# shichaoy/cube_slam

Hardware: AMD Instinct MI355X
Metric: frames/sec front-end (ORB extract + LSD+LBD lines + cuboid: Canny+DT+sweep+score+select) @640x480 (higher is better)
Workload: dtype f64

## Files before the change

### cube_slam_amd/csrc/cuboid.hip

```cpp
#include "common.h"

#include <algorithm>
#include <array>
#include <climits>
#include <cmath>
#include <vector>

namespace {

constexpr int ROLL_CAP = 8;
constexpr int RP_CAP = ROLL_CAP * ROLL_CAP;
constexpr int SWEEP_HB = 1024;
constexpr int NMS_TW = 64, NMS_TH = 16;
constexpr int DT_INIT = INT_MAX >> 2;
constexpr int DT_HV = 62587;
constexpr int DT_DIAG = 89738;
constexpr size_t DT_SERIAL_ROW_BYTES = 2 * 4 * sizeof(int);
constexpr double PI = 3.14159265358979323846;
constexpr int SC_LDS_BYTES = 160 * 1024;
constexpr int SC_LUT_N = 1024;
constexpr int SC_CTRL_BYTES = 64;
constexpr int SC_MAP_OFF = SC_CTRL_BYTES + 2048;
constexpr int SC_MAP_ENTRIES = (SC_LDS_BYTES - SC_MAP_OFF) / 2;
constexpr float SC_ESC_D = 244.0f;
// ... 824 lines not shown
}

__device__ __forceinline__ void hyp_decode(const Unit &U, int h, int &q, int &ti) {
    const unsigned p = (unsigned)h >> 1;
    q = U.tops_magic ? (int)__umulhi(p, U.tops_magic) : (int)(p / (unsigned)U.n_tops);
    ti = (int)p - q * U.n_tops;
}

__device__ __forceinline__ V2 hit_vertical(V2 ps, V2 pe, double bx, double by0, double by1) {
    const double dx = pe.x - ps.x, dy = pe.y - ps.y;
    const double lambd = (bx - ps.x) / dx;
    const double ty = ps.y + lambd * dy;
    const bool hit = lambd >= 0 && by0 <= ty && ty <= by1;
    return V2{hit ? bx : -1.0, hit ? ty : -1.0};
}
__device__ __forceinline__ V2 hit_horizontal(V2 ps, V2 pe, double by, double bx0, double bx1) {
    const double dx = pe.x - ps.x, dy = pe.y - ps.y;
    const double lambd = (by - ps.y) / dy;
    const double tx = ps.x + lambd * dx;
    const bool hit = lambd >= 0 && bx0 <= tx && tx <= bx1;
    return V2{hit ? tx : -1.0, hit ? by : -1.0};
}

template <bool TESTS, bool N78>
__device__ __forceinline__ int corners_build(const Unit &U, const double *vp, int top_x, int cfg, V2 (&c)[8], bool live = true) {
    auto short_edge = [](V2 a, V2 b) { const double dx = a.x - b.x, dy = a.y - b.y; return dx * dx + dy * dy < __longlong_as_double(0x4078ffffffffffffll); };
    const V2 vp_1{vp[0], vp[1]}, vp_2{vp[2], vp[3]}, vp_3{vp[4], vp[5]};
    const double left = U.left, right = U.right, top = U.top, down = U.down_y_expan;
    const V2 c1{(double)top_x, top};
    const V2 c2r = hit_vertical(vp_1, c1, right, top, down), c2l = hit_vertical(vp_1, c1, left, top, down);
    const int pos = c2r.x != -1 ? 1 : (c2l.x != -1 ? 2 : 0);
    const V2 c2 = pos == 1 ? c2r : c2l;
    bool alive = live && pos > 0;
    if (TESTS) { alive = alive && !short_edge(c1, c2); if (!__any(alive)) return 0; }
    const bool k1 = cfg == 1;
    const V2 S = k1 ? c1 : c2, other = k1 ? c2 : c1;
    const V2 X = hit_vertical(vp_2, S, pos == 1 ? left : right, top, down);
    if (TESTS) { alive = alive && X.y != -1 && !short_edge(S, X); if (!__any(alive)) return 0; }
    const V2 Y = k1 ? line_intersect_inf(vp_2, other, vp_1, X) : line_intersect_inf(vp_1, X, vp_2, other);
    if (TESTS) {
        alive = alive && inside_box(Y, left, k1 ? top : (double)U.roi_y, right, k1 ? down : (double)U.roi_b) && !short_edge(Y, X) && !short_edge(Y, other);
        if (!__any(alive)) return 0;
    }
    const V2 c3 = k1 ? Y : X, c4 = k1 ? X : Y;
    const double el = U.roi_x, et = U.roi_y, er = U.roi_r, eb = U.roi_b;
    const V2 c5 = hit_horizontal(vp_3, c3, down, left, right);
    if (TESTS) { alive = alive && c5.y != -1 && !short_edge(c3, c5); if (!__any(alive)) return 0; }
    const V2 c6 = line_intersect_inf(vp_2, c5, vp_3, c2);
    if (TESTS) { alive = alive && inside_box(c6, el, et, er, eb) && !short_edge(c6, c2) && !short_edge(c6, c5); if (!__any(alive)) return 0; }
    c[0] = c1; c[1] = c2; c[2] = c3; c[3] = c4; c[4] = c5; c[5] = c6;
    if (TESTS || N78) {
        const V2 c7 = line_intersect_inf(vp_1, c6, vp_3, c1);
        if (TESTS) { alive = alive && inside_box(c7, el, et, er, eb) && !short_edge(c7, c1) && !short_edge(c7, c6); if (!__any(alive)) return 0; }
        const V2 c8 = line_intersect_inf(vp_1, c5, vp_2, c7);
        if (TESTS) alive = alive && inside_box(c8, el, et, er, eb) && !short_edge(c8, c4) && !short_edge(c8, c5) && !short_edge(c8, c7);
        c[6] = c7; c[7] = c8;
    } else { c[6] = V2{0, 0}; c[7] = V2{0, 0}; }
    return alive ? pos : 0;
}

__global__ void __launch_bounds__(256) cuboid_sweep_filter(const Unit *units, const int *wg_unit, const FrameDyn *fd, Opts o,
                                                           const VPEntry *vpt, uint8_t *flag, int *vcount, int *vlist) {
    __shared__ int s_list[2][SWEEP_HB / 2];
    __shared__ int s_wc[2][SWEEP_HB / 64];
    __shared__ int s_base[2];
    const int u = __builtin_amdgcn_readfirstlane(wg_unit[blockIdx.x]);
    const Unit &U = units[u];
// ... 314 lines not shown
        k = s_misc[1];
    }
    return prefix;
}
template <class P, class F> __device__ int block_ordered_visit(int n, P pred, F cb, int *s_wave ) {
    const int lane = threadIdx.x & 63, wave = threadIdx.x >> 6, nw = blockDim.x >> 6;
    int running = 0;
    for (int base = 0; base < n; base += blockDim.x) {
        int i = base + threadIdx.x;
        bool p = i < n && pred(i);
        unsigned long long m = __ballot(p);
        if (lane == 0) s_wave[wave] = __popcll(m);
        __syncthreads();
        int off = running, tot = 0;
        for (int w2 = 0; w2 < nw; w2++) { int c = s_wave[w2]; if (w2 < wave) off += c; tot += c; }
        if (p) cb(i, off + __popcll(m & ((1ull << lane) - 1)));
        running += tot;
        __syncthreads();
    }
    return running;
}

struct Conv3D { double pos[3], scale[3]; };
__device__ inline void plane_hit(const double *T, const double *invK, const double *pl, double px, double py, double *o3) {
    double ray[3];
    for (int i = 0; i < 3; i++) {
        double s = invK[i * 3] * px;
        s = s + invK[i * 3 + 1] * py;
        s = s + invK[i * 3 + 2] * 1.0;
        ray[i] = s;
    }
    double den = pl[0] * ray[0];
    den = den + pl[1] * ray[1];
    den = den + pl[2] * ray[2];
    double frac = -pl[3] / den;
    double s4[4] = {frac * ray[0], frac * ray[1], frac * ray[2], 1.0};
    double w[4];
    for (int i = 0; i < 4; i++) {
        double a = T[i * 4] * s4[0];
        a = a + T[i * 4 + 1] * s4[1];
        a = a + T[i * 4 + 2] * s4[2];
        a = a + T[i * 4 + 3] * s4[3];
        w[i] = a;
    }
    o3[0] = w[0] / w[3]; o3[1] = w[1] / w[3]; o3[2] = w[2] / w[3];
}
__device__ inline void corners_to_3d(const double *cx, const double *cy, const CamRP &C, const double *invK, Conv3D &o) {
    double g[4][3];
    for (int i = 0; i < 4; i++) plane_hit(C.T, invK, C.gps, cx[4 + i], cy[4 + i], g[i]);
    auto nrm = [](const double *a, const double *b) {
        double dx = a[0] - b[0], dy = a[1] - b[1], dz = a[2] - b[2];
        return sqrt(dx * dx + dy * dy + dz * dz);
    };
    double length_half = nrm(g[0], g[3]) / 2;
    double width_half = nrm(g[0], g[1]) / 2;
    double d[3] = {g[0][0] - g[1][0], g[0][1] - g[1][1], g[0][2] - g[1][2]};
    double nw[3] = {d[1] * 1.0 - d[2] * 0.0, d[2] * 0.0 - d[0] * 1.0, d[0] * 0.0 - d[1] * 0.0};
    double nn = sqrt(nw[0] * nw[0] + nw[1] * nw[1] + nw[2] * nw[2]);
    nw[0] /= nn; nw[1] /= nn; nw[2] /= nn;
    double dist = -((nw[0] * g[0][0] + nw[1] * g[0][1]) + nw[2] * g[0][2]);
    double pw[4] = {nw[0], nw[1], nw[2], dist};
    if (dist < 0) for (int i = 0; i < 4; i++) pw[i] = -pw[i];
    double ps[4];
    for (int i = 0; i < 4; i++) {
        double s = C.T[0 * 4 + i] * pw[0];
        s = s + C.T[1 * 4 + i] * pw[1];
        s = s + C.T[2 * 4 + i] * pw[2];
        s = s + C.T[3 * 4 + i] * pw[3];
        ps[i] = s;
    }
    double top[3];
    plane_hit(C.T, invK, ps, cx[1], cy[1], top);
    double height_half = top[2] / 2;
    o.pos[0] = (((g[0][0] + g[1][0]) + g[2][0]) + g[3][0]) / 4.0;
    o.pos[1] = (((g[0][1] + g[1][1]) + g[2][1]) + g[3][1]) / 4.0;
    o.pos[2] = height_half;
    o.scale[0] = length_half; o.scale[1] = width_half; o.scale[2] = height_half;
}

#ifndef SELECT_WAVES
#define SELECT_WAVES 3
#endif
__global__ void __launch_bounds__(256) __attribute__((amdgpu_waves_per_eu(SELECT_WAVES, SELECT_WAVES))) cuboid_select(const Unit *units, UnitDyn *ud, const int *box_first_unit, const FrameDyn *fd,
                                                     const FrameInfo *fi, const CamRP *cam, const double *yaw, Calib cal, Opts o,
                                                     uint8_t *flag, const double *derr, const double *aerr, const VPEntry *vpt,
                                                     double *score, double *nscore, unsigned long long *ckey_d, unsigned long long *ckey_a,
                                                     int *cidx, cs_cuboid *out, int *counts, int *carry_rp) {
    __shared__ int hist[256];
    __shared__ int s_last;
    __shared__ int s_misc[8];
    __shared__ int s_wave[8];
    __shared__ double s_red[4][4];
    __shared__ double s_best[4];
    __shared__ int s_bi[4][2];
    __shared__ int s_branch[4];
    const int box = blockIdx.x, tid = threadIdx.x, lane = tid & 63, wave = tid >> 6;
    const int u0 = box_first_unit[box];
    const int n_hs = units[u0].n_hs;
    const FrameDyn &D = fd[units[u0].frame];
    const FrameInfo &FI = fi[units[u0].frame];
    const int n_rp = D.n_roll * D.n_pitch;
    const double weight_vp_angle = 0.8, weight_skew_error = 1.5;
    int n_cand_total = 0;

    for (int hs = 0; hs < n_hs; hs++) {
        const int u = u0 + hs;
        const Unit &U = units[u];
        const int n_hyp = n_rp * D.n_yaw * U.n_tops * 2;
        uint8_t *fl = flag + U.hyp_off;
        const double *de = derr + U.hyp_off, *ae = aerr + U.hyp_off;
        unsigned long long *ckd = ckey_d + U.hyp_off, *cka = ckey_a + U.hyp_off;
        int *ch = cidx + U.hyp_off;
        const int n = block_ordered_visit(n_hyp, [&](int i) { return fl[i] != 0; },
                                          [&](int i, int r) { ckd[r] = dkey(de[i]); cka[r] = dkey(ae[i]); ch[r] = i; }, s_wave);
        __syncthreads();
        KeyCache kd, ka;
#pragma unroll
        for (int k = 0; k < SEL_R; k++) { int e = tid + 256 * k; kd.v[k] = e < n ? ckd[e] : 0; ka.v[k] = e < n ? cka[e] : 0; }
        int branch_b = 0, n_kept = 0;
        if (tid == 0) s_last = n - 1;
        if (n > 4) {
            int breaking_num = (int)round(float(n) / 3.0 * 2.0);
            int k = breaking_num - 1;
            unsigned long long vd = block_select_kth(kd, ckd, n, k - 1, hist, s_misc);
            unsigned long long va = block_select_kth(ka, cka, n, k - 1, hist, s_misc);
            unsigned long long va1 = block_select_kth(ka, cka, n, k, hist, s_misc);
            __syncthreads();
            if (tid == 0) { s_misc[2] = 0; s_misc[3] = 0; s_misc[4] = INT_MAX; }
            __syncthreads();
            {
                int nl = 0, ne = 0;
                for_keys(kd, ckd, n, [&](unsigned long long key, int) { nl += key < vd; ne += key == vd; });
                for (int off = 32; off > 0; off >>= 1) { nl += __shfl_xor(nl, off); ne += __shfl_xor(ne, off); }
                if (lane == 0) { atomicAdd(&s_misc[2], nl); atomicAdd(&s_misc[3], ne); }
            }
            __syncthreads();
            const int need_eq = k - s_misc[2];
            if (need_eq < s_misc[3] && tid == 0) {
                int seen = 0;
                for (int e = 0; e < n; e++) if (ckd[e] == vd && ++seen == need_eq) { s_misc[4] = e; break; }
            }
            __syncthreads();
            const int e_star = s_misc[4];
            const bool use_angle = va1 > va;
            if (!use_angle) branch_b = 1;
#pragma unroll
            for (int kk = 0; kk < SEL_R; kk++) {
                int e = tid + 256 * kk;
                if (e < n) {
                    bool ok = kd.v[kk] < vd || (kd.v[kk] == vd && e <= e_star);
                    if (use_angle) ok = ok && ka.v[kk] <= va;
                    if (ok) fl[ch[e]] |= 4;
                }
            }
            for (int e = tid + 256 * SEL_R; e < n; e += 256) {
                bool ok = ckd[e] < vd || (ckd[e] == vd && e <= e_star);
                if (use_angle) ok = ok && cka[e] <= va;
                if (ok) fl[ch[e]] |= 4;
            }
            if (hs == n_hs - 1 && carry_rp) {
                __syncthreads();
                if (tid == 0) s_last = -1;
                __syncthreads();
                int mine = -1;
                for (int e = tid; e < n; e += 256) {
                    const bool kept = (ckd[e] < vd || (ckd[e] == vd && e <= e_star)) && (!use_angle || cka[e] <= va);
                    if (kept && (use_angle || ckd[e] == vd)) mine = e;
                }
                if (mine >= 0) atomicMax(&s_last, mine);
                __syncthreads();
            }
        } else {
            for (int e = tid; e < n; e += 256) fl[ch[e]] |= 4;
        }
        __syncthreads();
        if (hs == n_hs - 1 && carry_rp) {
            __syncthreads();
            if (tid == 0) {
                int rp = n_rp - 1;
                if (n > 0 && s_last >= 0) { int q, ti; hyp_decode(U, ch[s_last], q, ti); rp = q / D.n_yaw; }
                carry_rp[box] = rp;
            }
        }
        double mn_d = 1e6, mx_d = -1, mn_a = 1e6, mx_a = -1;
        int cntk = 0;
        for (int e = tid; e < n; e += 256) {
            const int i = ch[e];
            if (fl[i] & 4) {
                double td = de[i], ta = ae[i];
                mn_d = fmin(mn_d, td); mx_d = fmax(mx_d, td); mn_a = fmin(mn_a, ta); mx_a = fmax(mx_a, ta);
                cntk++;
            }
        }
        for (int off = 32; off > 0; off >>= 1) {
            mn_d = fmin(mn_d, __shfl_xor(mn_d, off)); mx_d = fmax(mx_d, __shfl_xor(mx_d, off));
            mn_a = fmin(mn_a, __shfl_xor(mn_a, off)); mx_a = fmax(mx_a, __shfl_xor(mx_a, off));
            cntk += __shfl_xor(cntk, off);
        }
        if (lane == 0) { s_red[wave][0] = mn_d; s_red[wave][1] = mx_d; s_red[wave][2] = mn_a; s_red[wave][3] = mx_a; s_wave[wave] = cntk; }
        __syncthreads();
        mn_d = fmin(fmin(s_red[0][0], s_red[1][0]), fmin(s_red[2][0], s_red[3][0]));
        mx_d = fmax(fmax(s_red[0][1], s_red[1][1]), fmax(s_red[2][1], s_red[3][1]));
        mn_a = fmin(fmin(s_red[0][2], s_red[1][2]), fmin(s_red[2][2], s_red[3][2]));
        mx_a = fmax(fmax(s_red[0][3], s_red[1][3]), fmax(s_red[2][3], s_red[3][3]));
        n_kept = s_wave[0] + s_wave[1] + s_wave[2] + s_wave[3];
        __syncthreads();
        int ncand = 0;
        for (int e = tid; e < n; e += 256) {
            const int i = ch[e];
            if (!(fl[i] & 4)) continue;
            double dk = de[i], ak = ae[i], comb;
            if (n_kept > 1) {
                comb = (dk - mn_d) / (mx_d - mn_d);
                if ((mx_a - mn_a) > 0) ak = (ak - mn_a) / (mx_a - mn_a);
                comb = (comb + weight_vp_angle * ak) / (1 + weight_vp_angle);
            } else
                comb = (dk + weight_vp_angle * ak) / (1 + weight_vp_angle);
            long g = U.hyp_off + i;
            int q, ti;
            hyp_decode(U, i, q, ti);
            int rp = q / D.n_yaw;
            double cx[8], cy[8];
            {
                V2 c[8];
                corners_build<false, true>(U, vpt[(long)U.vp_off + q].vp, U.top_start + ti * U.top_step, (i & 1) + 1, c);
                for (int k = 0; k < 8; k++) { cx[k] = c[k].x; cy[k] = c[k].y; }
            }
            Conv3D c3;
            corners_to_3d(cx, cy, cam[(long)U.frame * RP_CAP + rp], cal.invK, c3);
            if (c3.scale[0] < 0 || c3.scale[1] < 0 || c3.scale[2] < 0) continue;
            double mxs = c3.scale[0] < c3.scale[1] ? c3.scale[1] : c3.scale[0];
            double mns = c3.scale[1] < c3.scale[0] ? c3.scale[1] : c3.scale[0];
            double skew_ratio = mxs / mns;
            double dsk = skew_ratio - o.nominal_skew_ratio;
            double skew_error = weight_skew_error * ((dsk < 0.0) ? 0.0 : dsk);
            if (skew_ratio > o.max_cut_skew) skew_error = 100;
            nscore[g] = comb;
            score[g] = comb + weight_skew_error * skew_error;
            fl[i] |= 8;
            ncand++;
        }
        for (int off = 32; off > 0; off >>= 1) ncand += __shfl_xor(ncand, off);
        if (lane == 0) s_wave[wave] = ncand;
        __syncthreads();
        n_cand_total += s_wave[0] + s_wave[1] + s_wave[2] + s_wave[3];
        if (tid == 0) { ud[u].n_valid = n; ud[u].n_kept = n_kept; ud[u].branch_b = branch_b; s_branch[hs] = branch_b; }
        __syncthreads();
    }

    const int kout = n_cand_total < o.max_cuboid_num ? n_cand_total : o.max_cuboid_num;
    for (int pick = 0; pick < kout; pick++) {
        double bs = 0, bd = 0; int bhs = -1, bi = -1;
        for (int hs = 0; hs < n_hs; hs++) {
            const Unit &U = units[u0 + hs];
            const int n_hyp = n_rp * D.n_yaw * U.n_tops * 2;
            const uint8_t *fl = flag + U.hyp_off;
            const int bb = s_branch[hs];
            for (int i = tid; i < n_hyp; i += 256) {
                if (!(fl[i] & 8)) continue;
                double s = score[U.hyp_off + i], dd = bb ? derr[U.hyp_off + i] : 0.0;
                bool better = bi < 0 || s < bs || (s == bs && (hs < bhs || (hs == bhs && (dd < bd || (dd == bd && i < bi)))));
                if (better) { bs = s; bd = dd; bhs = hs; bi = i; }
            }
        }
        for (int off = 32; off > 0; off >>= 1) {
            double s2 = __shfl_xor(bs, off), d2 = __shfl_xor(bd, off);
            int hs2 = __shfl_xor(bhs, off), i2 = __shfl_xor(bi, off);
            bool better = i2 >= 0 && (bi < 0 || s2 < bs || (s2 == bs && (hs2 < bhs || (hs2 == bhs && (d2 < bd || (d2 == bd && i2 < bi))))));
            if (better) { bs = s2; bd = d2; bhs = hs2; bi = i2; }
        }
        if (lane == 0) { s_best[wave] = bs; s_red[wave][0] = bd; s_bi[wave][0] = bhs; s_bi[wave][1] = bi; }
        __syncthreads();
        if (tid == 0) {
            for (int w2 = 1; w2 < 4; w2++) {
                double s2 = s_best[w2], d2 = s_red[w2][0];
                int hs2 = s_bi[w2][0], i2 = s_bi[w2][1];
                bool better = i2 >= 0 && (bi < 0 || s2 < bs || (s2 == bs && (hs2 < bhs || (hs2 == bhs && (d2 < bd || (d2 == bd && i2 < bi))))));
                if (better) { bs = s2; bd = d2; bhs = hs2; bi = i2; }
            }
            const Unit &U = units[u0 + bhs];
            long g = U.hyp_off + bi;
            flag[g] &= ~8;
            int cfg = (bi & 1) + 1, q, ti;
            hyp_decode(U, bi, q, ti);
            int yi = q % D.n_yaw, rp = q / D.n_yaw;
            const CamRP &C = cam[(long)U.frame * RP_CAP + rp];
            double cx[8], cy[8];
            {
                V2 c[8];
                corners_build<false, true>(U, vpt[(long)U.vp_off + q].vp, U.top_start + ti * U.top_step, cfg, c);
                for (int k = 0; k < 8; k++) { cx[k] = c[k].x; cy[k] = c[k].y; }
            }
            Conv3D c3;
            corners_to_3d(cx, cy, C, cal.invK, c3);
            cs_cuboid &O = out[(long)box * o.max_cuboid_num + pick];
            for (int k = 0; k < 3; k++) { O.pos[k] = c3.pos[k]; O.scale[k] = c3.scale[k]; }
            O.rotY = yaw[(long)U.frame * o.yaw_cap + yi];
            int vp1 = flag[g] & 3;
            O.box_config_type[0] = cfg; O.box_config_type[1] = vp1;
            const int map1[8] = {6, 5, 8, 7, 2, 3, 4, 1}, map2[8] = {5, 6, 7, 8, 3, 2, 1, 4};
            for (int k = 0; k < 8; k++) {
                int src = (vp1 == 1 ? map1[k] : map2[k]) - 1;
// ... 17 lines not shown
                    for (int i = 0; i < 3; i++) {
                        double s = rs[i][0] * body[0][k];
                        s = s + rs[i][1] * body[1][k];
                        s = s + rs[i][2] * body[2][k];
                        s = s + O.pos[i] * 1.0;
                        wv[i] = s;
                    }
                    wv[3] = ((0.0 * body[0][k] + 0.0 * body[1][k]) + 0.0 * body[2][k]) + 1.0;
                    for (int i = 0; i < 3; i++) O.box_corners_3d_world[i * 8 + k] = wv[i] / wv[3];
                }
            }
            O.rect_detect_2d[0] = U.left; O.rect_detect_2d[1] = U.top; O.rect_detect_2d[2] = U.width_raw; O.rect_detect_2d[3] = U.height_raw;
            O.edge_distance_error = derr[g]; O.edge_angle_error = aerr[g];
            O.normalized_error = nscore[g];
            double mxs = c3.scale[0] < c3.scale[1] ? c3.scale[1] : c3.scale[0];
            double mns = c3.scale[1] < c3.scale[0] ? c3.scale[1] : c3.scale[0];
            O.skew_ratio = mxs / mns;
            O.down_expand_height = U.down_expand;
            if (o.sample_rp) { O.camera_roll_delta = C.roll - FI.euler[0]; O.camera_pitch_delta = C.pitch - FI.euler[1]; }
            else { O.camera_roll_delta = 0; O.camera_pitch_delta = 0; }
        }
        __syncthreads();
    }
    if (tid == 0) counts[box] = kout;
}

__global__ void cuboid_bgr2gray(const uint8_t *bgr, int stride, int w, int h, uint8_t *gray) {
    int x = blockIdx.x * blockDim.x + threadIdx.x, y = blockIdx.y;
    if (x >= w) return;
    const uint8_t *p = bgr + (long)y * stride + 3 * x;
    gray[(long)y * w + x] = (uint8_t)((p[0] * 1868 + p[1] * 9617 + p[2] * 4899 + 8192) >> 14);
}

static void host_euler_from_T(const double *T, double *euler) {
    double m[3][3];
    for (int i = 0; i < 3; i++) for (int j = 0; j < 3; j++) m[i][j] = T[i * 4 + j];
    double qw, qx, qy, qz, q[3];
    double t = m[0][0] + m[1][1] + m[2][2];
    if (t > 0) {
        t = std::sqrt(t + 1.0);
        qw = 0.5 * t; t = 0.5 / t;
        qx = (m[2][1] - m[1][2]) * t; qy = (m[0][2] - m[2][0]) * t; qz = (m[1][0] - m[0][1]) * t;
    } else {
        int i = 0;
        if (m[1][1] > m[0][0]) i = 1;
        if (m[2][2] > m[i][i]) i = 2;
        int j = (i + 1) % 3, k = (j + 1) % 3;
// ... 140 lines not shown
    cs_pinned<uint8_t> stage[2]; hipEvent_t stage_ev[2] = {nullptr, nullptr}; int stage_k = 0;
    hipEvent_t ev_fork = nullptr, ev_join = nullptr;
    int score_G = 256;
    int score_T = 512;
    bool score_T_forced = false;
    bool want_carry = false;
    uint8_t *d_gray = nullptr;
    FrameInfo *d_fi = nullptr; FrameDyn *d_fd = nullptr; CamRP *d_cam = nullptr;
    double *d_yaw = nullptr;
    int *d_status = nullptr, *d_cursor = nullptr;
    uint8_t *d_emap = nullptr, *d_flag = nullptr;
    float *d_dist = nullptr;
    int *d_lab = nullptr;
    int *d_dttmp = nullptr; long *d_dttmp_off = nullptr;
    int *d_wgmap = nullptr;
    int *d_order = nullptr;
    int *d_uflag = nullptr;
    double *d_lines_in = nullptr, *d_lines_al = nullptr, *d_mlines = nullptr, *d_mangle = nullptr, *d_mmid = nullptr;
    Unit *d_units = nullptr; UnitDyn *d_ud = nullptr; int *d_box_first = nullptr, *d_counts = nullptr, *d_carry = nullptr;
    VPEntry *d_vp = nullptr;
    int *d_vcount = nullptr, *d_vlist = nullptr;
    double *d_derr = nullptr, *d_aerr = nullptr, *d_score = nullptr, *d_nscore = nullptr;
    unsigned long long *d_ckd = nullptr, *d_cka = nullptr; int *d_cidx = nullptr;
    cs_cuboid *d_out = nullptr;
    cs_cuboid_batch() { cap.fill(-1); }
};
static void plan_commit(cs_cuboid_batch *b, Plan &P) { static_cast<Plan &>(*b) = std::move(P); }

struct BatchArray { void **slot; int cls; size_t elem, mul, add; };
template <class T> static BatchArray array_of(T *&p, int cls, size_t mul = 1, size_t add = 0) { return {reinterpret_cast<void **>(&p), cls, sizeof(T), mul, add}; }
constexpr size_t N_BATCH_ARRAYS = 29;
static std::array<BatchArray, N_BATCH_ARRAYS> batch_arrays(cs_cuboid_batch *b) {
    return {{array_of(b->d_emap, K_PIX, 1, 256),
             array_of(b->d_dist, K_PIX),
             array_of(b->d_flag, K_HYP), array_of(b->d_vlist, K_HYP), array_of(b->d_derr, K_HYP), array_of(b->d_aerr, K_HYP), array_of(b->d_score, K_HYP), array_of(b->d_nscore, K_HYP),
             array_of(b->d_ckd, K_HYP), array_of(b->d_cka, K_HYP), array_of(b->d_cidx, K_HYP),
             array_of(b->d_vp, K_VP),
             array_of(b->d_units, K_UNITS), array_of(b->d_ud, K_UNITS), array_of(b->d_order, K_UNITS), array_of(b->d_uflag, K_UNITS), array_of(b->d_vcount, K_UNITS, 2),
             array_of(b->d_dttmp_off, K_UNITS, 1, 1),
             array_of(b->d_box_first, K_BOXES), array_of(b->d_counts, K_BOXES), array_of(b->d_carry, K_BOXES), array_of(b->d_out, K_BOXES, (size_t)b->o.max_cuboid_num),
             array_of(b->d_lines_in, K_LINES_IN, 4), array_of(b->d_lines_al, K_LINES_IN, 4),
             array_of(b->d_mlines, K_LINE_ROWS, 4), array_of(b->d_mangle, K_LINE_ROWS), array_of(b->d_mmid, K_LINE_ROWS, 2),
             array_of(b->d_wgmap, K_WGMAP),
             array_of(b->d_dttmp, K_DTTMP)}};
}
static int batch_reserve(cs_ctx *ctx, cs_cuboid_batch *b, const Needs &need, bool exact) {
    Needs cap = b->cap;
    for (int c = 0; c < K_N; c++)
        if (need[c] > cap[c]) cap[c] = exact ? need[c] : need[c] + need[c] / 4 + (c == K_LINES_IN || c == K_LINE_ROWS ? 64 : 0);
    if (cap == b->cap) return CS_OK;
    const auto arrays = batch_arrays(b);
    cs_owner fresh;
    std::array<uint8_t *, N_BATCH_ARRAYS> blk{};
    for (size_t i = 0; i < arrays.size(); i++) {
        const BatchArray &A = arrays[i];
        if (cap[A.cls] == b->cap[A.cls]) continue;
        const int r = fresh.alloc(ctx, &blk[i], std::max<size_t>(1, (size_t)cap[A.cls] * A.mul + A.add) * A.elem);
        if (r != CS_OK) { fresh.free_all(ctx); return r; }
    }
    bool replaces = false;
    for (size_t i = 0; i < arrays.size(); i++) replaces |= blk[i] && *arrays[i].slot;
    const hipError_t e = replaces ? ctx->drain() : hipSuccess;
// ... 213 lines not shown
    if (fork) { CS_HIP(ctx, hipEventRecord(b->ev_join, side)); branch.joined = b->ev_join; }
    CS_HIP(ctx, hipMemsetAsync(b->d_emap, 0, (size_t)b->pix_total, ctx->stream));
    CS_LAUNCH(ctx, "cuboid_canny_nms", cuboid_canny_nms, dim3(b->n_nms), dim3(256), 0, b->d_units, b->d_wgmap, b->d_gray, b->W, b->H, b->d_emap,
              b->d_lab, b->o.canny_low, b->o.canny_high);
    CS_LAUNCH(ctx, "cuboid_canny_cc_local", cuboid_canny_cc_local, dim3(b->n_cc), dim3(256), 0, b->d_units, b->d_wgmap + b->n_nms, b->d_emap, b->d_lab);
    if (b->max_cc_blocks > 1)
        CS_LAUNCH(ctx, "cuboid_canny_cc_border", cuboid_canny_cc_border, dim3(U, 4), dim3(256), 0, b->d_units, b->d_emap, b->d_lab);
    CS_LAUNCH(ctx, "cuboid_canny_cc", cuboid_canny_cc, dim3(b->n_cc), dim3(256), 0, b->d_units, b->d_wgmap + b->n_nms, b->d_emap, b->d_lab);
    if (b->dt_C) {
        const dim3 g((U + 3) / 4), t(256);
        switch (b->dt_C) {
#define DTW_(c) case c: CS_LAUNCH(ctx, "cuboid_dt", cuboid_dt_wave<c>, g, t, 0, b->d_units, U, b->d_emap, b->d_dttmp, b->d_dttmp_off, b->d_dist); break;
            DTW_(4) DTW_(5) DTW_(6) DTW_(8) DTW_(10) DTW_(12) DTW_(16) DTW_(20)
#undef DTW_
        }
    } else if (b->max_roi_w <= 1024) {
        CS_LAUNCH(ctx, "cuboid_dt", cuboid_dt_block, dim3(U), dim3(64 * ((b->max_roi_w + 63) / 64)), 0, b->d_units, b->d_emap, b->d_dist);
    } else {
        const int wbuf = b->max_roi_w + 2;
        CS_LAUNCH(ctx, "cuboid_dt", cuboid_dt, dim3((U + 3) / 4), dim3(256), (size_t)wbuf * DT_SERIAL_ROW_BYTES, b->d_units, U, b->d_emap, b->d_dist, wbuf);
    }
    CS_HIP(ctx, branch.join());
    CS_HIP(ctx, hipMemsetAsync(b->d_vcount, 0, sizeof(int) * 2 * (size_t)U, ctx->stream));
    CS_LAUNCH(ctx, "cuboid_sweep_filter", cuboid_sweep_filter, dim3(b->n_hb), dim3(256), 0, b->d_units, b->d_wgmap + b->n_nms + b->n_cc, b->d_fd, b->o, b->d_vp,
              b->d_flag, b->d_vcount, b->d_vlist);
    CS_HIP(ctx, hipMemsetAsync(b->d_cursor, 0, sizeof(int), ctx->stream));
    CS_HIP(ctx, hipMemsetAsync(b->d_uflag, 0, sizeof(int) * (size_t)U, ctx->stream));
    {
        const int items = U * b->score_slices, grid = std::min(b->score_G, items);
        switch (b->score_T) {
#define SCORE_(nt) case nt: CS_LAUNCH(ctx, "cuboid_sweep_score", cuboid_sweep_score<nt>, dim3(grid), dim3(nt), SC_LDS_BYTES, b->d_units, b->d_order, items, b->score_slices, b->d_cursor, b->d_vp, \
                                      b->d_dist, b->d_vcount, b->d_vlist, b->d_uflag, b->d_derr, b->d_aerr); break;
            SCORE_(256) SCORE_(512) SCORE_(768) SCORE_(1024)
#undef SCORE_
        }
    }
    CS_LAUNCH(ctx, "cuboid_select", cuboid_select, dim3(b->n_boxes), dim3(256), 0, b->d_units, b->d_ud, b->d_box_first, b->d_fd, b->d_fi,
              b->d_cam, b->d_yaw, b->cal, b->o, b->d_flag, b->d_derr, b->d_aerr, b->d_vp, b->d_score, b->d_nscore,
              b->d_ckd, b->d_cka, b->d_cidx, b->d_out, b->d_counts, b->want_carry ? b->d_carry : nullptr);
    CS_HIP(ctx, hipGetLastError());
    return CS_OK;
}

int cs_cuboid_batch_read(cs_ctx *ctx, cs_cuboid_batch *b, cs_cuboid *out, int *counts) {
    if (!ctx || !b || !out || !counts) return CS_ERR_BAD_ARG;
    int status = 0;
    int r = cs_d2h(ctx, out, b->d_out, (size_t)b->n_boxes * b->o.max_cuboid_num); if (r) return r;
    r = cs_d2h(ctx, counts, b->d_counts, (size_t)b->n_boxes); if (r) return r;
    r = cs_d2h(ctx, &status, b->d_status, 1); if (r) return r;
    CS_HIP(ctx, hipStreamSynchronize(ctx->stream));
    if (status != 0) { ctx->err = "more than CS_MAX_ROI_LINES lines inside one box"; return status; }
    return CS_OK;
}

int cs_cuboid_batch_read_on(cs_cuboid_batch *b, void *stream, cs_cuboid *out, int *counts, int *status_out) {
    if (!b || !out || !counts || !status_out) return CS_ERR_BAD_ARG;
    hipStream_t s = (hipStream_t)stream;
    if (hipMemcpyAsync(out, b->d_out, sizeof(cs_cuboid) * (size_t)b->n_boxes * b->o.max_cuboid_num, hipMemcpyDeviceToHost, s) != hipSuccess ||
        hipMemcpyAsync(counts, b->d_counts, sizeof(int) * (size_t)b->n_boxes, hipMemcpyDeviceToHost, s) != hipSuccess ||
        hipMemcpyAsync(status_out, b->d_status, sizeof(int), hipMemcpyDeviceToHost, s) != hipSuccess) return CS_ERR_HIP;
    return CS_OK;
}
// ... 160 lines not shown
```

Measured before the change: 28360.

## Split cuboid select into per-unit keep, chunked cost, and per-box pick kernels

Replaces the single per-box cuboid_select kernel, which looped serially over height-sample units, with three kernels. A per-unit keep kernel computes the kth-threshold and the extents, a 2D-grid cost kernel builds corners and 3D scale penalties in parallel chunks, and a single-wave pick kernel chooses the best candidates by scanning only the compacted candidate list. It also swaps the third kth-select for a count-based test on the angle threshold, force-inlines and unrolls the 3D conversion helpers, and skips the sweep-filter launch when there is no work. In exchange it adds two extra launches and global intermediates (ext, ncand), and the pick now runs with one wave instead of four.

```diff
diff --git a/cube_slam_amd/csrc/cuboid.hip b/cube_slam_amd/csrc/cuboid.hip
--- a/cube_slam_amd/csrc/cuboid.hip
+++ b/cube_slam_amd/csrc/cuboid.hip
@@ -870,7 +870,7 @@
     return V2{hit ? tx : -1.0, hit ? by : -1.0};
 }
 
-template <bool TESTS, bool N78>
+template <bool TESTS, bool N78, bool PICKED = false>
 __device__ __forceinline__ int corners_build(const Unit &U, const double *vp, int top_x, int cfg, V2 (&c)[8], bool live = true) {
     auto short_edge = [](V2 a, V2 b) { const double dx = a.x - b.x, dy = a.y - b.y; return dx * dx + dy * dy < __longlong_as_double(0x4078ffffffffffffll); };
     const V2 vp_1{vp[0], vp[1]}, vp_2{vp[2], vp[3]}, vp_3{vp[4], vp[5]};
@@ -885,12 +885,14 @@
     const V2 S = k1 ? c1 : c2, other = k1 ? c2 : c1;
     const V2 X = hit_vertical(vp_2, S, pos == 1 ? left : right, top, down);
     if (TESTS) { alive = alive && X.y != -1 && !short_edge(S, X); if (!__any(alive)) return 0; }
-    const V2 Y = k1 ? line_intersect_inf(vp_2, other, vp_1, X) : line_intersect_inf(vp_1, X, vp_2, other);
+    auto pick2 = [](bool c, V2 a, V2 b) { return V2{c ? a.x : b.x, c ? a.y : b.y}; };
+    const V2 Y = PICKED ? line_intersect_inf(pick2(k1, vp_2, vp_1), pick2(k1, other, X), pick2(k1, vp_1, vp_2), pick2(k1, X, other))
+                        : (k1 ? line_intersect_inf(vp_2, other, vp_1, X) : line_intersect_inf(vp_1, X, vp_2, other));
     if (TESTS) {
         alive = alive && inside_box(Y, left, k1 ? top : (double)U.roi_y, right, k1 ? down : (double)U.roi_b) && !short_edge(Y, X) && !short_edge(Y, other);
         if (!__any(alive)) return 0;
     }
-    const V2 c3 = k1 ? Y : X, c4 = k1 ? X : Y;
+    const V2 c3 = PICKED ? pick2(k1, Y, X) : (k1 ? Y : X), c4 = PICKED ? pick2(k1, X, Y) : (k1 ? X : Y);
     const double el = U.roi_x, et = U.roi_y, er = U.roi_r, eb = U.roi_b;
     const V2 c5 = hit_horizontal(vp_3, c3, down, left, right);
     if (TESTS) { alive = alive && c5.y != -1 && !short_edge(c3, c5); if (!__any(alive)) return 0; }
@@ -1251,8 +1253,9 @@
 }
 
 struct Conv3D { double pos[3], scale[3]; };
-__device__ inline void plane_hit(const double *T, const double *invK, const double *pl, double px, double py, double *o3) {
+__device__ __forceinline__ void plane_hit(const double *T, const double *invK, const double *pl, double px, double py, double *o3) {
     double ray[3];
+#pragma unroll
     for (int i = 0; i < 3; i++) {
         double s = invK[i * 3] * px;
         s = s + invK[i * 3 + 1] * py;
@@ -1265,6 +1268,7 @@
     double frac = -pl[3] / den;
     double s4[4] = {frac * ray[0], frac * ray[1], frac * ray[2], 1.0};
     double w[4];
+#pragma unroll
     for (int i = 0; i < 4; i++) {
         double a = T[i * 4] * s4[0];
         a = a + T[i * 4 + 1] * s4[1];
@@ -1274,8 +1278,9 @@
     }
     o3[0] = w[0] / w[3]; o3[1] = w[1] / w[3]; o3[2] = w[2] / w[3];
 }
-__device__ inline void corners_to_3d(const double *cx, const double *cy, const CamRP &C, const double *invK, Conv3D &o) {
+__device__ __forceinline__ void corners_to_3d(const double *cx, const double *cy, const CamRP &C, const double *invK, Conv3D &o) {
     double g[4][3];
+#pragma unroll
     for (int i = 0; i < 4; i++) plane_hit(C.T, invK, C.gps, cx[4 + i], cy[4 + i], g[i]);
     auto nrm = [](const double *a, const double *b) {
         double dx = a[0] - b[0], dy = a[1] - b[1], dz = a[2] - b[2];
@@ -1291,6 +1296,7 @@
     double pw[4] = {nw[0], nw[1], nw[2], dist};
     if (dist < 0) for (int i = 0; i < 4; i++) pw[i] = -pw[i];
     double ps[4];
+#pragma unroll
     for (int i = 0; i < 4; i++) {
         double s = C.T[0 * 4 + i] * pw[0];
         s = s + C.T[1 * 4 + i] * pw[1];
@@ -1307,185 +1313,210 @@
     o.scale[0] = length_half; o.scale[1] = width_half; o.scale[2] = height_half;
 }
 
-#ifndef SELECT_WAVES
-#define SELECT_WAVES 3
-#endif
-__global__ void __launch_bounds__(256) __attribute__((amdgpu_waves_per_eu(SELECT_WAVES, SELECT_WAVES))) cuboid_select(const Unit *units, UnitDyn *ud, const int *box_first_unit, const FrameDyn *fd,
-                                                     const FrameInfo *fi, const CamRP *cam, const double *yaw, Calib cal, Opts o,
-                                                     uint8_t *flag, const double *derr, const double *aerr, const VPEntry *vpt,
-                                                     double *score, double *nscore, unsigned long long *ckey_d, unsigned long long *ckey_a,
-                                                     int *cidx, cs_cuboid *out, int *counts, int *carry_rp) {
+__device__ __forceinline__ double dkey_inv(unsigned long long k) {
+    return __longlong_as_double((long long)((k >> 63) ? (k & 0x7fffffffffffffffull) : ~k));
+}
+constexpr int SEL_COST_CHUNKS = 8;
+
+__global__ void __launch_bounds__(256) __attribute__((amdgpu_waves_per_eu(4))) cuboid_select_keep(const Unit *units, UnitDyn *ud, const FrameDyn *fd, uint8_t *flag, const double *derr, const double *aerr,
+                                                          unsigned long long *ckey_d, unsigned long long *ckey_a, int *cidx, double *ext, int *ncand, int *carry_rp) {
     __shared__ int hist[256];
     __shared__ int s_last;
     __shared__ int s_misc[8];
     __shared__ int s_wave[8];
     __shared__ double s_red[4][4];
-    __shared__ double s_best[4];
-    __shared__ int s_bi[4][2];
-    __shared__ int s_branch[4];
-    const int box = blockIdx.x, tid = threadIdx.x, lane = tid & 63, wave = tid >> 6;
+    const int u = blockIdx.x, tid = threadIdx.x, lane = tid & 63, wave = tid >> 6;
+    const Unit &U = units[u];
+    const FrameDyn &D = fd[U.frame];
+    const int n_rp = D.n_roll * D.n_pitch;
+    const int n_hyp = n_rp * D.n_yaw * U.n_tops * 2;
+    const bool carry = U.hs == U.n_hs - 1 && carry_rp;
+    uint8_t *fl = flag + U.hyp_off;
+    const double *de = derr + U.hyp_off, *ae = aerr + U.hyp_off;
+    unsigned long long *ckd = ckey_d + U.hyp_off, *cka = ckey_a + U.hyp_off;
+    int *ch = cidx + U.hyp_off;
+    const int n = block_ordered_visit(n_hyp, [&](int i) { return fl[i] != 0; },
+                                      [&](int i, int r) { ckd[r] = dkey(de[i]); cka[r] = dkey(ae[i]); ch[r] = i; }, s_wave);
+    __syncthreads();
+    KeyCache kd, ka;
+#pragma unroll
+    for (int k = 0; k < SEL_R; k++) { int e = tid + 256 * k; kd.v[k] = e < n ? ckd[e] : 0; ka.v[k] = e < n ? cka[e] : 0; }
+    int branch_b = 0;
+    unsigned long long vd = 0, va = 0;
+    int e_star = INT_MAX;
+    bool use_angle = false;
+    if (tid == 0) s_last = n - 1;
+    if (n > 4) {
+        int breaking_num = (int)round(float(n) / 3.0 * 2.0);
+        int k = breaking_num - 1;
+        vd = block_select_kth(kd, ckd, n, k - 1, hist, s_misc);
+        va = block_select_kth(ka, cka, n, k - 1, hist, s_misc);
+        __syncthreads();
+        if (tid == 0) { s_misc[2] = 0; s_misc[3] = 0; s_misc[4] = INT_MAX; s_misc[5] = 0; }
+        __syncthreads();
+        {
+            int nl = 0, ne = 0, na = 0;
+#pragma unroll
+            for (int kk = 0; kk < SEL_R; kk++) {
+                const int e = tid + 256 * kk;
+                if (e < n) { nl += kd.v[kk] < vd; ne += kd.v[kk] == vd; na += ka.v[kk] <= va; }
+            }
+            for (int e = tid + 256 * SEL_R; e < n; e += 256) { const unsigned long long d = ckd[e]; nl += d < vd; ne += d == vd; na += cka[e] <= va; }
+            for (int off = 32; off > 0; off >>= 1) { nl += __shfl_xor(nl, off); ne += __shfl_xor(ne, off); na += __shfl_xor(na, off); }
+            if (lane == 0) { atomicAdd(&s_misc[2], nl); atomicAdd(&s_misc[3], ne); atomicAdd(&s_misc[5], na); }
+        }
+        __syncthreads();
+        const int need_eq = k - s_misc[2];
+        if (need_eq < s_misc[3] && tid == 0) {
+            int seen = 0;
+            for (int e = 0; e < n; e++) if (ckd[e] == vd && ++seen == need_eq) { s_misc[4] = e; break; }
+        }
+        __syncthreads();
+        e_star = s_misc[4];
+        use_angle = s_misc[5] == k;
+        if (!use_angle) branch_b = 1;
+        if (carry) {
+            __syncthreads();
+            if (tid == 0) s_last = -1;
+            __syncthreads();
+            int mine = -1;
+            for (int e = tid; e < n; e += 256) {
+                const bool kept = (ckd[e] < vd || (ckd[e] == vd && e <= e_star)) && (!use_angle || cka[e] <= va);
+                if (kept && (use_angle || ckd[e] == vd)) mine = e;
+            }
+            if (mine >= 0) atomicMax(&s_last, mine);
+            __syncthreads();
+        }
+    }
+    __syncthreads();
+    if (carry && tid == 0) {
+        int rp = n_rp - 1;
+        if (n > 0 && s_last >= 0) { int q, ti; hyp_decode(U, ch[s_last], q, ti); rp = q / D.n_yaw; }
+        carry_rp[U.box] = rp;
+    }
+    double mn_d = 1e6, mx_d = -1, mn_a = 1e6, mx_a = -1;
+    int cntk = 0;
+    auto take = [&](unsigned long long d, unsigned long long a, int e) {
+        bool ok = true;
+        if (n > 4) {
+            ok = d < vd || (d == vd && e <= e_star);
+            if (use_angle) ok = ok && a <= va;
+        }
+        if (ok) {
+            fl[ch[e]] |= 4;
+            const double td = dkey_inv(d), ta = dkey_inv(a);
+            mn_d = fmin(mn_d, td); mx_d = fmax(mx_d, td); mn_a = fmin(mn_a, ta); mx_a = fmax(mx_a, ta);
+            cntk++;
+        }
+    };
+#pragma unroll
+    for (int kk = 0; kk < SEL_R; kk++) { const int e = tid + 256 * kk; if (e < n) take(kd.v[kk], ka.v[kk], e); }
+    for (int e = tid + 256 * SEL_R; e < n; e += 256) take(ckd[e], cka[e], e);
+    for (int off = 32; off > 0; off >>= 1) {
+        mn_d = fmin(mn_d, __shfl_xor(mn_d, off)); mx_d = fmax(mx_d, __shfl_xor(mx_d, off));
+        mn_a = fmin(mn_a, __shfl_xor(mn_a, off)); mx_a = fmax(mx_a, __shfl_xor(mx_a, off));
+        cntk += __shfl_xor(cntk, off);
+    }
+    if (lane == 0) { s_red[wave][0] = mn_d; s_red[wave][1] = mx_d; s_red[wave][2] = mn_a; s_red[wave][3] = mx_a; s_wave[wave] = cntk; }
+    __syncthreads();
+    if (tid == 0) {
+        ext[4 * (long)u + 0] = fmin(fmin(s_red[0][0], s_red[1][0]), fmin(s_red[2][0], s_red[3][0]));
+        ext[4 * (long)u + 1] = fmax(fmax(s_red[0][1], s_red[1][1]), fmax(s_red[2][1], s_red[3][1]));
+        ext[4 * (long)u + 2] = fmin(fmin(s_red[0][2], s_red[1][2]), fmin(s_red[2][2], s_red[3][2]));
+        ext[4 * (long)u + 3] = fmax(fmax(s_red[0][3], s_red[1][3]), fmax(s_red[2][3], s_red[3][3]));
+        ud[u].n_valid = n; ud[u].n_kept = s_wave[0] + s_wave[1] + s_wave[2] + s_wave[3]; ud[u].branch_b = branch_b;
+        ncand[u] = 0;
+    }
+}
+
+__device__ __forceinline__ bool select_cost_one(const Unit &U, const CamRP &C, const VPEntry *vpt, const Calib &cal, const Opts &o, int i, int q, int ti, double &penalty) {
+    const double weight_skew_error = 1.5;
+    double cx[8], cy[8];
+    {
+        V2 c[8];
+        corners_build<false, true, true>(U, vpt[(long)U.vp_off + q].vp, U.top_start + ti * U.top_step, (i & 1) + 1, c);
+#pragma unroll
+        for (int k = 0; k < 8; k++) { cx[k] = c[k].x; cy[k] = c[k].y; }
+    }
+    Conv3D c3;
+    corners_to_3d(cx, cy, C, cal.invK, c3);
+    if (c3.scale[0] < 0 || c3.scale[1] < 0 || c3.scale[2] < 0) return false;
+    double mxs = c3.scale[0] < c3.scale[1] ? c3.scale[1] : c3.scale[0];
+    double mns = c3.scale[1] < c3.scale[0] ? c3.scale[1] : c3.scale[0];
+    double skew_ratio = mxs / mns;
+    double dsk = skew_ratio - o.nominal_skew_ratio;
+    double skew_error = weight_skew_error * ((dsk < 0.0) ? 0.0 : dsk);
+    if (skew_ratio > o.max_cut_skew) skew_error = 100;
+    penalty = weight_skew_error * skew_error;
+    return true;
+}
+
+__global__ void __launch_bounds__(64) __attribute__((amdgpu_waves_per_eu(4))) cuboid_select_cost(const Unit *units, const UnitDyn *ud, const FrameDyn *fd, const CamRP *cam, Calib cal, Opts o,
+                                                         uint8_t *flag, const double *derr, const double *aerr, const VPEntry *vpt, const int *cidx, const double *ext,
+                                                         double *score, double *nscore, int *ncand) {
+    const int u = blockIdx.y, lane = threadIdx.x;
+    const int n = ud[u].n_valid, n_kept = ud[u].n_kept;
+    if ((int)blockIdx.x * 64 >= n) return;
+    const Unit &U = units[u];
+    const FrameDyn &D = fd[U.frame];
+    const bool one_rp = D.n_roll * D.n_pitch == 1;
+    const CamRP *camf = cam + (long)U.frame * RP_CAP;
+    const double weight_vp_angle = 0.8;
+    const double mn_d = ext[4 * (long)u + 0], mx_d = ext[4 * (long)u + 1], mn_a = ext[4 * (long)u + 2], mx_a = ext[4 * (long)u + 3];
+    uint8_t *fl = flag + U.hyp_off;
+    const double *de = derr + U.hyp_off, *ae = aerr + U.hyp_off;
+    const int *ch = cidx + U.hyp_off;
+    int cnt = 0;
+    for (int e0 = (int)blockIdx.x * 64; e0 < n; e0 += SEL_COST_CHUNKS * 64) {
+        const int e = e0 + lane;
+        bool cand = false;
+        if (e < n) {
+            const int i = ch[e];
+            if (fl[i] & 4) {
+                double dk = de[i], ak = ae[i], comb;
+                if (n_kept > 1) {
+                    comb = (dk - mn_d) / (mx_d - mn_d);
+                    if ((mx_a - mn_a) > 0) ak = (ak - mn_a) / (mx_a - mn_a);
+                    comb = (comb + weight_vp_angle * ak) / (1 + weight_vp_angle);
+                } else
+                    comb = (dk + weight_vp_angle * ak) / (1 + weight_vp_angle);
+                int q, ti;
+                hyp_decode(U, i, q, ti);
+                double penalty = 0;
+                cand = one_rp ? select_cost_one(U, camf[0], vpt, cal, o, i, q, ti, penalty) : select_cost_one(U, camf[q / D.n_yaw], vpt, cal, o, i, q, ti, penalty);
+                if (cand) {
+                    const long g = U.hyp_off + i;
+                    nscore[g] = comb;
+                    score[g] = comb + penalty;
+                    fl[i] |= 8;
+                }
+            }
+        }
+        cnt += __popcll(__ballot(cand));
+    }
+    if (lane == 0 && cnt) atomicAdd(&ncand[u], cnt);
+}
+
+__global__ void __launch_bounds__(64) __attribute__((amdgpu_waves_per_eu(4))) cuboid_select_pick(const Unit *units, const UnitDyn *ud, const int *box_first_unit, const FrameDyn *fd, const FrameInfo *fi,
+                                                         const CamRP *cam, const double *yaw, Calib cal, Opts o, uint8_t *flag, const double *derr, const double *aerr,
+                                                         const VPEntry *vpt, const double *score, const double *nscore, const int *cidx, const int *ncand, cs_cuboid *out, int *counts) {
+    const int box = blockIdx.x, lane = threadIdx.x;
     const int u0 = box_first_unit[box];
     const int n_hs = units[u0].n_hs;
     const FrameDyn &D = fd[units[u0].frame];
     const FrameInfo &FI = fi[units[u0].frame];
-    const int n_rp = D.n_roll * D.n_pitch;
-    const double weight_vp_angle = 0.8, weight_skew_error = 1.5;
     int n_cand_total = 0;
-
-    for (int hs = 0; hs < n_hs; hs++) {
-        const int u = u0 + hs;
-        const Unit &U = units[u];
-        const int n_hyp = n_rp * D.n_yaw * U.n_tops * 2;
-        uint8_t *fl = flag + U.hyp_off;
-        const double *de = derr + U.hyp_off, *ae = aerr + U.hyp_off;
-        unsigned long long *ckd = ckey_d + U.hyp_off, *cka = ckey_a + U.hyp_off;
-        int *ch = cidx + U.hyp_off;
-        const int n = block_ordered_visit(n_hyp, [&](int i) { return fl[i] != 0; },
-                                          [&](int i, int r) { ckd[r] = dkey(de[i]); cka[r] = dkey(ae[i]); ch[r] = i; }, s_wave);
-        __syncthreads();
-        KeyCache kd, ka;
-#pragma unroll
-        for (int k = 0; k < SEL_R; k++) { int e = tid + 256 * k; kd.v[k] = e < n ? ckd[e] : 0; ka.v[k] = e < n ? cka[e] : 0; }
-        int branch_b = 0, n_kept = 0;
-        if (tid == 0) s_last = n - 1;
-        if (n > 4) {
-            int breaking_num = (int)round(float(n) / 3.0 * 2.0);
-            int k = breaking_num - 1;
-            unsigned long long vd = block_select_kth(kd, ckd, n, k - 1, hist, s_misc);
-            unsigned long long va = block_select_kth(ka, cka, n, k - 1, hist, s_misc);
-            unsigned long long va1 = block_select_kth(ka, cka, n, k, hist, s_misc);
-            __syncthreads();
-            if (tid == 0) { s_misc[2] = 0; s_misc[3] = 0; s_misc[4] = INT_MAX; }
-            __syncthreads();
-            {
-                int nl = 0, ne = 0;
-                for_keys(kd, ckd, n, [&](unsigned long long key, int) { nl += key < vd; ne += key == vd; });
-                for (int off = 32; off > 0; off >>= 1) { nl += __shfl_xor(nl, off); ne += __shfl_xor(ne, off); }
-                if (lane == 0) { atomicAdd(&s_misc[2], nl); atomicAdd(&s_misc[3], ne); }
-            }
-            __syncthreads();
-            const int need_eq = k - s_misc[2];
-            if (need_eq < s_misc[3] && tid == 0) {
-                int seen = 0;
-                for (int e = 0; e < n; e++) if (ckd[e] == vd && ++seen == need_eq) { s_misc[4] = e; break; }
-            }
-            __syncthreads();
-            const int e_star = s_misc[4];
-            const bool use_angle = va1 > va;
-            if (!use_angle) branch_b = 1;
-#pragma unroll
-            for (int kk = 0; kk < SEL_R; kk++) {
-                int e = tid + 256 * kk;
-                if (e < n) {
-                    bool ok = kd.v[kk] < vd || (kd.v[kk] == vd && e <= e_star);
-                    if (use_angle) ok = ok && ka.v[kk] <= va;
-                    if (ok) fl[ch[e]] |= 4;
-                }
-            }
-            for (int e = tid + 256 * SEL_R; e < n; e += 256) {
-                bool ok = ckd[e] < vd || (ckd[e] == vd && e <= e_star);
-                if (use_angle) ok = ok && cka[e] <= va;
-                if (ok) fl[ch[e]] |= 4;
-            }
-            if (hs == n_hs - 1 && carry_rp) {
-                __syncthreads();
-                if (tid == 0) s_last = -1;
-                __syncthreads();
-                int mine = -1;
-                for (int e = tid; e < n; e += 256) {
-                    const bool kept = (ckd[e] < vd || (ckd[e] == vd && e <= e_star)) && (!use_angle || cka[e] <= va);
-                    if (kept && (use_angle || ckd[e] == vd)) mine = e;
-                }
-                if (mine >= 0) atomicMax(&s_last, mine);
-                __syncthreads();
-            }
-        } else {
-            for (int e = tid; e < n; e += 256) fl[ch[e]] |= 4;
-        }
-        __syncthreads();
-        if (hs == n_hs - 1 && carry_rp) {
-            __syncthreads();
-            if (tid == 0) {
-                int rp = n_rp - 1;
-                if (n > 0 && s_last >= 0) { int q, ti; hyp_decode(U, ch[s_last], q, ti); rp = q / D.n_yaw; }
-                carry_rp[box] = rp;
-            }
-        }
-        double mn_d = 1e6, mx_d = -1, mn_a = 1e6, mx_a = -1;
-        int cntk = 0;
-        for (int e = tid; e < n; e += 256) {
-            const int i = ch[e];
-            if (fl[i] & 4) {
-                double td = de[i], ta = ae[i];
-                mn_d = fmin(mn_d, td); mx_d = fmax(mx_d, td); mn_a = fmin(mn_a, ta); mx_a = fmax(mx_a, ta);
-                cntk++;
-            }
-        }
-        for (int off = 32; off > 0; off >>= 1) {
-            mn_d = fmin(mn_d, __shfl_xor(mn_d, off)); mx_d = fmax(mx_d, __shfl_xor(mx_d, off));
-            mn_a = fmin(mn_a, __shfl_xor(mn_a, off)); mx_a = fmax(mx_a, __shfl_xor(mx_a, off));
-            cntk += __shfl_xor(cntk, off);
-        }
-        if (lane == 0) { s_red[wave][0] = mn_d; s_red[wave][1] = mx_d; s_red[wave][2] = mn_a; s_red[wave][3] = mx_a; s_wave[wave] = cntk; }
-        __syncthreads();
-        mn_d = fmin(fmin(s_red[0][0], s_red[1][0]), fmin(s_red[2][0], s_red[3][0]));
-        mx_d = fmax(fmax(s_red[0][1], s_red[1][1]), fmax(s_red[2][1], s_red[3][1]));
-        mn_a = fmin(fmin(s_red[0][2], s_red[1][2]), fmin(s_red[2][2], s_red[3][2]));
-        mx_a = fmax(fmax(s_red[0][3], s_red[1][3]), fmax(s_red[2][3], s_red[3][3]));
-        n_kept = s_wave[0] + s_wave[1] + s_wave[2] + s_wave[3];
-        __syncthreads();
-        int ncand = 0;
-        for (int e = tid; e < n; e += 256) {
-            const int i = ch[e];
-            if (!(fl[i] & 4)) continue;
-            double dk = de[i], ak = ae[i], comb;
-            if (n_kept > 1) {
-                comb = (dk - mn_d) / (mx_d - mn_d);
-                if ((mx_a - mn_a) > 0) ak = (ak - mn_a) / (mx_a - mn_a);
-                comb = (comb + weight_vp_angle * ak) / (1 + weight_vp_angle);
-            } else
-                comb = (dk + weight_vp_angle * ak) / (1 + weight_vp_angle);
-            long g = U.hyp_off + i;
-            int q, ti;
-            hyp_decode(U, i, q, ti);
-            int rp = q / D.n_yaw;
-            double cx[8], cy[8];
-            {
-                V2 c[8];
-                corners_build<false, true>(U, vpt[(long)U.vp_off + q].vp, U.top_start + ti * U.top_step, (i & 1) + 1, c);
-                for (int k = 0; k < 8; k++) { cx[k] = c[k].x; cy[k] = c[k].y; }
-            }
-            Conv3D c3;
-            corners_to_3d(cx, cy, cam[(long)U.frame * RP_CAP + rp], cal.invK, c3);
-            if (c3.scale[0] < 0 || c3.scale[1] < 0 || c3.scale[2] < 0) continue;
-            double mxs = c3.scale[0] < c3.scale[1] ? c3.scale[1] : c3.scale[0];
-            double mns = c3.scale[1] < c3.scale[0] ? c3.scale[1] : c3.scale[0];
-            double skew_ratio = mxs / mns;
-            double dsk = skew_ratio - o.nominal_skew_ratio;
-            double skew_error = weight_skew_error * ((dsk < 0.0) ? 0.0 : dsk);
-            if (skew_ratio > o.max_cut_skew) skew_error = 100;
-            nscore[g] = comb;
-            score[g] = comb + weight_skew_error * skew_error;
-            fl[i] |= 8;
-            ncand++;
-        }
-        for (int off = 32; off > 0; off >>= 1) ncand += __shfl_xor(ncand, off);
-        if (lane == 0) s_wave[wave] = ncand;
-        __syncthreads();
-        n_cand_total += s_wave[0] + s_wave[1] + s_wave[2] + s_wave[3];
-        if (tid == 0) { ud[u].n_valid = n; ud[u].n_kept = n_kept; ud[u].branch_b = branch_b; s_branch[hs] = branch_b; }
-        __syncthreads();
-    }
-
+    for (int hs = 0; hs < n_hs; hs++) n_cand_total += ncand[u0 + hs];
     const int kout = n_cand_total < o.max_cuboid_num ? n_cand_total : o.max_cuboid_num;
     for (int pick = 0; pick < kout; pick++) {
         double bs = 0, bd = 0; int bhs = -1, bi = -1;
         for (int hs = 0; hs < n_hs; hs++) {
             const Unit &U = units[u0 + hs];
-            const int n_hyp = n_rp * D.n_yaw * U.n_tops * 2;
             const uint8_t *fl = flag + U.hyp_off;
-            const int bb = s_branch[hs];
-            for (int i = tid; i < n_hyp; i += 256) {
+            const int *ch = cidx + U.hyp_off;
+            const int n = ud[u0 + hs].n_valid, bb = ud[u0 + hs].branch_b;
+            for (int e = lane; e < n; e += 64) {
+                const int i = ch[e];
                 if (!(fl[i] & 8)) continue;
                 double s = score[U.hyp_off + i], dd = bb ? derr[U.hyp_off + i] : 0.0;
                 bool better = bi < 0 || s < bs || (s == bs && (hs < bhs || (hs == bhs && (dd < bd || (dd == bd && i < bi)))));
@@ -1498,15 +1529,7 @@
             bool better = i2 >= 0 && (bi < 0 || s2 < bs || (s2 == bs && (hs2 < bhs || (hs2 == bhs && (d2 < bd || (d2 == bd && i2 < bi))))));
             if (better) { bs = s2; bd = d2; bhs = hs2; bi = i2; }
         }
-        if (lane == 0) { s_best[wave] = bs; s_red[wave][0] = bd; s_bi[wave][0] = bhs; s_bi[wave][1] = bi; }
-        __syncthreads();
-        if (tid == 0) {
-            for (int w2 = 1; w2 < 4; w2++) {
-                double s2 = s_best[w2], d2 = s_red[w2][0];
-                int hs2 = s_bi[w2][0], i2 = s_bi[w2][1];
-                bool better = i2 >= 0 && (bi < 0 || s2 < bs || (s2 == bs && (hs2 < bhs || (hs2 == bhs && (d2 < bd || (d2 == bd && i2 < bi))))));
-                if (better) { bs = s2; bd = d2; bhs = hs2; bi = i2; }
-            }
+        if (lane == 0) {
             const Unit &U = units[u0 + bhs];
             long g = U.hyp_off + bi;
             flag[g] &= ~8;
@@ -1570,7 +1593,7 @@
         }
         __syncthreads();
     }
-    if (tid == 0) counts[box] = kout;
+    if (lane == 0) counts[box] = kout;
 }
 
 __global__ void cuboid_bgr2gray(const uint8_t *bgr, int stride, int w, int h, uint8_t *gray) {
@@ -1757,6 +1780,7 @@
     int *d_vcount = nullptr, *d_vlist = nullptr;
     double *d_derr = nullptr, *d_aerr = nullptr, *d_score = nullptr, *d_nscore = nullptr;
     unsigned long long *d_ckd = nullptr, *d_cka = nullptr; int *d_cidx = nullptr;
+    double *d_ext = nullptr; int *d_ncand = nullptr;
     cs_cuboid *d_out = nullptr;
     cs_cuboid_batch() { cap.fill(-1); }
 };
@@ -1764,7 +1788,7 @@
 
 struct BatchArray { void **slot; int cls; size_t elem, mul, add; };
 template <class T> static BatchArray array_of(T *&p, int cls, size_t mul = 1, size_t add = 0) { return {reinterpret_cast<void **>(&p), cls, sizeof(T), mul, add}; }
-constexpr size_t N_BATCH_ARRAYS = 29;
+constexpr size_t N_BATCH_ARRAYS = 31;
 static std::array<BatchArray, N_BATCH_ARRAYS> batch_arrays(cs_cuboid_batch *b) {
     return {{array_of(b->d_emap, K_PIX, 1, 256),
              array_of(b->d_dist, K_PIX),
@@ -1772,7 +1796,7 @@
              array_of(b->d_ckd, K_HYP), array_of(b->d_cka, K_HYP), array_of(b->d_cidx, K_HYP),
              array_of(b->d_vp, K_VP),
              array_of(b->d_units, K_UNITS), array_of(b->d_ud, K_UNITS), array_of(b->d_order, K_UNITS), array_of(b->d_uflag, K_UNITS), array_of(b->d_vcount, K_UNITS, 2),
-             array_of(b->d_dttmp_off, K_UNITS, 1, 1),
+             array_of(b->d_dttmp_off, K_UNITS, 1, 1), array_of(b->d_ext, K_UNITS, 4), array_of(b->d_ncand, K_UNITS),
              array_of(b->d_box_first, K_BOXES), array_of(b->d_counts, K_BOXES), array_of(b->d_carry, K_BOXES), array_of(b->d_out, K_BOXES, (size_t)b->o.max_cuboid_num),
              array_of(b->d_lines_in, K_LINES_IN, 4), array_of(b->d_lines_al, K_LINES_IN, 4),
              array_of(b->d_mlines, K_LINE_ROWS, 4), array_of(b->d_mangle, K_LINE_ROWS), array_of(b->d_mmid, K_LINE_ROWS, 2),
@@ -2032,8 +2056,9 @@
     }
     CS_HIP(ctx, branch.join());
     CS_HIP(ctx, hipMemsetAsync(b->d_vcount, 0, sizeof(int) * 2 * (size_t)U, ctx->stream));
-    CS_LAUNCH(ctx, "cuboid_sweep_filter", cuboid_sweep_filter, dim3(b->n_hb), dim3(256), 0, b->d_units, b->d_wgmap + b->n_nms + b->n_cc, b->d_fd, b->o, b->d_vp,
-              b->d_flag, b->d_vcount, b->d_vlist);
+    if (b->n_hb)
+        CS_LAUNCH(ctx, "cuboid_sweep_filter", cuboid_sweep_filter, dim3(b->n_hb), dim3(256), 0, b->d_units, b->d_wgmap + b->n_nms + b->n_cc, b->d_fd, b->o, b->d_vp,
+                  b->d_flag, b->d_vcount, b->d_vlist);
     CS_HIP(ctx, hipMemsetAsync(b->d_cursor, 0, sizeof(int), ctx->stream));
     CS_HIP(ctx, hipMemsetAsync(b->d_uflag, 0, sizeof(int) * (size_t)U, ctx->stream));
     {
@@ -2045,9 +2070,12 @@
 #undef SCORE_
         }
     }
-    CS_LAUNCH(ctx, "cuboid_select", cuboid_select, dim3(b->n_boxes), dim3(256), 0, b->d_units, b->d_ud, b->d_box_first, b->d_fd, b->d_fi,
-              b->d_cam, b->d_yaw, b->cal, b->o, b->d_flag, b->d_derr, b->d_aerr, b->d_vp, b->d_score, b->d_nscore,
-              b->d_ckd, b->d_cka, b->d_cidx, b->d_out, b->d_counts, b->want_carry ? b->d_carry : nullptr);
+    CS_LAUNCH(ctx, "cuboid_select", cuboid_select_keep, dim3(U), dim3(256), 0, b->d_units, b->d_ud, b->d_fd, b->d_flag, b->d_derr, b->d_aerr, b->d_ckd, b->d_cka, b->d_cidx,
+              b->d_ext, b->d_ncand, b->want_carry ? b->d_carry : nullptr);
+    CS_LAUNCH(ctx, "cuboid_select", cuboid_select_cost, dim3(SEL_COST_CHUNKS, U), dim3(64), 0, b->d_units, b->d_ud, b->d_fd, b->d_cam, b->cal, b->o, b->d_flag, b->d_derr, b->d_aerr, b->d_vp,
+              b->d_cidx, b->d_ext, b->d_score, b->d_nscore, b->d_ncand);
+    CS_LAUNCH(ctx, "cuboid_select", cuboid_select_pick, dim3(b->n_boxes), dim3(64), 0, b->d_units, b->d_ud, b->d_box_first, b->d_fd, b->d_fi, b->d_cam, b->d_yaw, b->cal, b->o,
+              b->d_flag, b->d_derr, b->d_aerr, b->d_vp, b->d_score, b->d_nscore, b->d_cidx, b->d_ncand, b->d_out, b->d_counts);
     CS_HIP(ctx, hipGetLastError());
     return CS_OK;
 }
```

After: 28240. Within noise of the previous version (-0.4%).
